# Kirkice/3DGaussian

Measured on AMD Instinct MI355X. Metric: Mpixels/sec fwd+bwd @1M Gaussians 800×800; PSNR vs torch ref, higher is better.
Workload: dtype f32 (splat contractions on v_mfma_f32_32x32x16_f16 with f32 accumulation; every operand in two round-to-nearest f16 pieces, pre-scaled into f16's normal range, three piece products: <= 3*2^-22 per product, forward and backward; no-depth-gradient mode); 1 GPU; C4: 1000000 Gaussians, 50 orbit views 800x800, fwd+bwd+grad all-reduce+Adam per step; gaussians=1000000, views=50, width=800, height=800, tile=32, seed=0, parallelism=view-sharded dp1, gaussian_order=morton (trainer layout, re-established every 16 steps)

## Files before the change

### 3dgaussian_amd/csrc/gr_hip.hip

```cpp

#include <hip/hip_runtime.h>
#include <hipcub/hipcub.hpp>
#include <rocprim/rocprim.hpp>

#include <cmath>
#include <cstdint>
#include <cstdio>
#include <cstdlib>
#include <cstring>
#include <atomic>
#include <mutex>
#include <string>
#include <vector>

#include "../../include/gr_hip.h"

#ifndef GR_TAIL2
#define GR_TAIL2 1
#endif
#ifndef GR_DEBUG_PREP_REPS
#define GR_DEBUG_PREP_REPS 1
#endif
#ifndef GR_DEBUG_BIN_REPS
#define GR_DEBUG_BIN_REPS 1
// ... 165 lines not shown
#pragma unroll
      for (int i = 4; i < 16; ++i)
#pragma unroll
        for (int k = 0; k < 3; ++k) out[k] += col[3 * i + k] * Y[i];
    }
  }
}

__device__ __forceinline__ float clamp01(float x) { return x < 0.0f ? 0.0f : (x > 1.0f ? 1.0f : x); }

__device__ __forceinline__ int tile_rect(const ViewK& v, const Proj& p, float op, int4& r) {
  r = make_int4(0, 0, -1, -1);
  if (!p.valid || !(op >= 0.0f)) return 0;
  const float R = v.cutoff;
  const float rx = R * p.sx, ry = R * p.sy;
  const float lox = p.px - rx, hix = p.px + rx, loy = p.py - ry, hiy = p.py + ry;
  const float wm1 = (float)(v.W - 1), hm1 = (float)(v.H - 1);
  if (!(hix >= 0.0f) || !(lox <= wm1) || !(hiy >= 0.0f) || !(loy <= hm1)) return 0;
  const int x0 = (lox <= 0.0f) ? 0 : (int)floorf(lox);
  const int x1 = (hix >= wm1) ? (v.W - 1) : (int)ceilf(hix);
  const int y0 = (loy <= 0.0f) ? 0 : (int)floorf(loy);
  const int y1 = (hiy >= hm1) ? (v.H - 1) : (int)ceilf(hiy);
  r = make_int4(x0 >> v.ts, y0 >> v.ts, x1 >> v.ts, y1 >> v.ts);
  r.y = max(r.y, v.ty0);
  r.w = min(r.w, v.ty1 - 1);
  if (r.y > r.w) {
    r = make_int4(0, 0, -1, -1);
    return 0;
  }
  return (r.z - r.x + 1) * (r.w - r.y + 1);
}

__device__ __forceinline__ float tile_emax(const ViewK& v, float px, float py, float qx, float qy, int tx, int ty) {
  const int xe = min(tx * v.T + v.T - 1, v.W - 1), ye = min(ty * v.T + v.T - 1, v.H - 1);
  const float lox = (float)(tx * v.T) + 0.5f, hix = (float)xe + 0.5f;
  const float loy = (float)(ty * v.T) + 0.5f, hiy = (float)ye + 0.5f;
  const float cx = px < lox ? lox : (px > hix ? hix : px);
  const float cy = py < loy ? loy : (py > hiy ? hiy : py);
  const float dx = cx - px, dy = cy - py;
  return (dx * dx) * qx + (dy * dy) * qy;
}

__device__ __forceinline__ float radius_thr(float R) { return (-0.5f * LOG2E) * (R * R); }

__device__ __forceinline__ float tile_ex(const ViewK& v, float px, float qx, int tx) {
  const int xe = min(tx * v.T + v.T - 1, v.W - 1);
  const float lox = (float)(tx * v.T) + 0.5f, hix = (float)xe + 0.5f;
  const float cx = px < lox ? lox : (px > hix ? hix : px);
  const float dx = cx - px;
  return (dx * dx) * qx;
}
__device__ __forceinline__ float tile_ey(const ViewK& v, float py, float qy, int ty) {
  const int ye = min(ty * v.T + v.T - 1, v.H - 1);
  const float loy = (float)(ty * v.T) + 0.5f, hiy = (float)ye + 0.5f;
  const float cy = py < loy ? loy : (py > hiy ? hiy : py);
  const float dy = cy - py;
  return (dy * dy) * qy;
}
__device__ __forceinline__ int tile_class_e(float e, float thr_cut, float thr_core) {
  return !(e >= thr_cut) ? 0 : (e >= thr_core ? 2 : 1);
}

__device__ __forceinline__ bool tile_pass(const ViewK& v, float px, float py, float qx, float qy, int tx, int ty) {
  return tile_emax(v, px, py, qx, qy, tx, ty) >= radius_thr(v.cutoff);
}

__device__ __forceinline__ int tile_class(const ViewK& v, float px, float py, float qx, float qy, int tx, int ty) {
  const float e = tile_emax(v, px, py, qx, qy, tx, ty);
  if (!(e >= radius_thr(v.cutoff))) return 0;
  return e >= radius_thr(v.core) ? 2 : 1;
}

__device__ __forceinline__ float qcoef(float s) { return (-0.5f * LOG2E) / (s * s); }


constexpr int REC4 = 2;

struct Cnt2 {
  unsigned long long v;
  __host__ __device__ unsigned c() const { return (unsigned)(v & 0xffffffffull); }
  __host__ __device__ unsigned t() const { return (unsigned)(v >> 32); }
};

struct Geom {
  float4* rec;
  float* zr;
  int4* rect;
  unsigned long long* counts;
  unsigned long long* offsets;
  gr_plan* plan;
  unsigned long long* total;
  float* omax;
  int* f16_sa;
  void* scan_tmp;
  size_t scan_tmp_bytes;
};

size_t geom_fixed(int n, size_t off[GR_GEOM_PARTS]) {
  size_t o = 0;
  const size_t nn = (size_t)(n > 0 ? n : 1);
  off[0] = o; o = align_up(o + (nn + 1) * (REC4 * sizeof(float4) + sizeof(float)));
  off[1] = o; o = align_up(o + nn * sizeof(int4));
  off[2] = o; o = align_up(o + (nn + 1) * sizeof(unsigned long long));
  off[3] = o; o = align_up(o + (nn + 1) * sizeof(unsigned long long));
  off[4] = o; o = align_up(o + sizeof(gr_plan) + (nn / 256 + 2) * (sizeof(unsigned long long) + sizeof(float)) + 16);
  off[5] = o;
  return o;
}

template <typename CountT>
size_t scan_tmp_bytes_t(int n) {
  size_t tmp = 0;
  (void)hipcub::DeviceScan::ExclusiveSum(nullptr, tmp, (CountT*)nullptr, (CountT*)nullptr, n + 1, (hipStream_t)0);
  return tmp;
}
size_t scan_tmp_bytes(int n) { return scan_tmp_bytes_t<unsigned long long>(n); }

Geom geom_view(void* base, int n) {
  size_t off[GR_GEOM_PARTS];
  const size_t fixed = geom_fixed(n, off);
  char* b = (char*)base;
  Geom g;
  g.plan = (gr_plan*)(b + off[4]);
  g.rec = (float4*)(b + off[0]);
  g.zr = (float*)(g.rec + (size_t)REC4 * ((size_t)n + 1));
  g.rect = (int4*)(b + off[1]);
  g.counts = (unsigned long long*)(b + off[2]);
  g.offsets = (unsigned long long*)(b + off[3]);
  g.total = (unsigned long long*)(b + off[4] + sizeof(gr_plan));
  g.omax = (float*)(g.total + (size_t)n / 256 + 2);
  g.f16_sa = (int*)(g.omax + (size_t)n / 256 + 2);
  g.scan_tmp = b + fixed;
  g.scan_tmp_bytes = 0;
  return g;
}

#ifndef GR_CH
#define GR_CH 2048
#endif
constexpr int CH = GR_CH;
#ifndef GR_CH32
#define GR_CH32 2048
#endif
constexpr int CH32 = GR_CH32;
constexpr int NPART = 9;

constexpr int TSORT_MAX_TILES = 16384;

inline bool short_keys(int tiles) { return tiles <= TSORT_MAX_TILES; }

struct Bins {
  uint32_t* keys;
  int* pairs;
  int2* ranges;
  int4* items;
  int* num_items;
  int* tile_item0;
  int* pos_of;
  int* ticket;
};

struct Scratch {
  uint32_t* keys_in;
  int* ids_in;
  float* fwd_part;
  int2* pairs_in;
  int2* pairs_sorted;
  void* sort_tmp;
};

inline int64_t item_cap(int tiles, int64_t K, int ch = CH) { return (K + ch - 1) / ch + tiles; }
constexpr int UF32_FRAGS = 2 * 4 * 2 * 2 * 64;
constexpr int UF32_STRIDE = UF32_FRAGS + 64;
struct TileCfg {
  int T, ch;
  size_t part_floats, uf_frags;
};
constexpr int UF_FRAGS16 = 2 * 3 * 3 * 64;
static int64_t tune_env(const char* name);
inline int chunk_of(const gr_view* v, int base, int64_t K) {
  static const int64_t force = tune_env("GR_TUNE_CHUNK");
  int64_t c = base;
  if (v->chunk > 0) {
    c = v->chunk;
  } else if (force > 0) {
    c = force;
  } else if (K >= 0) {
    c = 512;
    while (c < base && 2 * c * 1024 <= K) c *= 2;
  }
  return (int)std::min<int64_t>(8192, std::max<int64_t>(64, (c + 63) / 64 * 64));
}
inline TileCfg tile_cfg(const gr_view* v, int64_t K = -1) {
  return tile_of(v) == T32 ? TileCfg{T32, chunk_of(v, CH32, K), (size_t)4 * TP32, (size_t)UF32_STRIDE}
                           : TileCfg{T, chunk_of(v, CH, K), (size_t)5 * TP, (size_t)UF_FRAGS16};
}

constexpr int FAN_STRIDE = 32;
__host__ __device__ inline size_t fan_offset(int tiles) { return ((size_t)tiles + 1 + FAN_STRIDE - 1) / FAN_STRIDE * FAN_STRIDE; }

size_t bins_fixed(int vtiles, int64_t K, size_t off[8], int ch = CH) {
  const int tiles = vtiles;
  const size_t kk = (size_t)(K > 0 ? K : 1);
  const size_t cap = (size_t)item_cap(tiles, K, ch);
  size_t o = 0;
  off[0] = o; o = align_up(o + (short_keys(tiles) ? 1 : kk) * sizeof(uint32_t));
  off[1] = o; o = align_up(o + kk * sizeof(int));
  off[2] = o; o = align_up(o + (size_t)tiles * sizeof(int2));
  off[3] = o; o = align_up(o + cap * sizeof(int4));
  off[4] = o; o = align_up(o + 2 * sizeof(int));
  off[5] = o; o = align_up(o + (size_t)tiles * sizeof(int));
// ... 92 lines not shown
  r.keys_in = (uint32_t*)(b + off[0]);
  r.ids_in = (int*)(b + off[1]);
  r.fwd_part = (float*)(b + off[2]);
  r.pairs_in = (int2*)(b + off[3]);
  r.pairs_sorted = (int2*)(b + off[4]);
  r.sort_tmp = b + fixed;
  return r;
}

template <int NW>
__device__ __forceinline__ unsigned long long block_exclusive_scan(unsigned long long x, unsigned long long* sh,
                                                                   unsigned long long& total) {
  const int lane = (int)threadIdx.x & 63, w = (int)threadIdx.x >> 6;
  unsigned long long inc = x;
#pragma unroll
  for (int o = 1; o < 64; o <<= 1) {
    const unsigned long long y = __shfl_up(inc, o);
    if (lane >= o) inc += y;
  }
  __syncthreads();
  if (lane == 63) sh[w] = inc;
  __syncthreads();
  unsigned long long base = 0, all = 0;
#pragma unroll
  for (int u = 0; u < NW; ++u) {
    base += u < w ? sh[u] : 0ull;
    all += sh[u];
  }
  total = all;
  return base + inc - x;
}

template <int CD>
__device__ __forceinline__ unsigned long long preprocess_one(const ViewK& v, int i, const float* __restrict__ means,
                                                             const float* __restrict__ scales,
                                                             const float* __restrict__ colors,
                                                             const float* __restrict__ opac, Geom& g);

template <int CD>
__global__ __launch_bounds__(256) void k_preprocess(ViewK v, int n, const float* __restrict__ means,
                                                    const float* __restrict__ scales, const float* __restrict__ colors,
                                                    const float* __restrict__ opac, Geom g) {
  const int i = blockIdx.x * blockDim.x + threadIdx.x;
  if (i == n) {
    g.counts[n] = 0ull;
    float4* pad = g.rec + (size_t)REC4 * n;
    pad[0] = make_float4(1e30f, 1e30f, -1.0f, -1.0f);
    pad[1] = make_float4(0.f, 0.f, 0.f, 0.f);
    g.zr[n] = 0.0f;
  }
  unsigned long long kept = 0;
  if (i < n) kept = preprocess_one<CD>(v, i, means, scales, colors, opac, g);
  float om = kept != 0 ? g.rec[(size_t)REC4 * i + 1].x * fmaxf(1.0f, g.zr[i]) : 0.0f;
  __shared__ unsigned long long wsum[4];
  __shared__ float wmax[4];
#pragma unroll
  for (int m = 1; m < 64; m <<= 1) {
    kept += __shfl_xor(kept, m);
    om = fmaxf(om, __shfl_xor(om, m));
  }
  if ((threadIdx.x & 63) == 0) {
    wsum[threadIdx.x >> 6] = kept;
    wmax[threadIdx.x >> 6] = om;
  }
  __syncthreads();
  if (threadIdx.x == 0) {
    g.total[blockIdx.x] = (wsum[0] + wsum[1]) + (wsum[2] + wsum[3]);
    g.omax[blockIdx.x] = fmaxf(fmaxf(wmax[0], wmax[1]), fmaxf(wmax[2], wmax[3]));
  }
}

template <int CD>
__device__ __forceinline__ unsigned long long preprocess_vals(const ViewK& v, int i, float mx, float my, float mz, float s0,
                                                              float s1, const float* __restrict__ col, float op,
                                                              const Geom& g) {
  Proj p;
  project(v, mx, my, mz, s0, s1, p);
  float c[3];
  eval_color<CD>(v, mx, my, mz, col, c);
  int4 r;
  const float qx = qcoef(p.sx);
  const float qy = qcoef(p.sy);
  int core = 0, tail = 0;
  const int area = tile_rect(v, p, op, r);
  if (area > 0) {
    const float thr_cut = radius_thr(v.cutoff), thr_core = radius_thr(v.core);
    for (int ty = r.y; ty <= r.w; ++ty) {
      const float ey = tile_ey(v, p.py, qy, ty);
      for (int tx = r.x; tx <= r.z; ++tx) {
        const int cls = tile_class_e(tile_ex(v, p.px, qx, tx) + ey, thr_cut, thr_core);
        core += cls == 2;
        tail += cls == 1;
      }
    }
  }
  float4* rec = g.rec + (size_t)REC4 * i;
  rec[0] = make_float4(p.px, p.py, qx, qy);
  rec[1] = make_float4(op < 0.0f ? 0.0f : op, clamp01(c[0]), clamp01(c[1]), clamp01(c[2]));
  g.zr[i] = p.za;
  g.rect[i] = r;
  g.counts[i] = (unsigned long long)core | ((unsigned long long)tail << 32);
  return (unsigned long long)core | ((unsigned long long)tail << 32);
}

template <int CD>
__device__ __forceinline__ unsigned long long preprocess_one(const ViewK& v, int i, const float* __restrict__ means,
                                                             const float* __restrict__ scales,
                                                             const float* __restrict__ colors,
                                                             const float* __restrict__ opac, Geom& g) {
  return preprocess_vals<CD>(v, i, means[3 * i], means[3 * i + 1], means[3 * i + 2], scales[3 * i], scales[3 * i + 1],
                             colors + (size_t)CD * i, opac[i], g);
}

constexpr int PREP_MAX_VIEWS = GR_PREPARE_MAX_VIEWS;
struct PrepBatch {
  int nv;
  ViewK v[PREP_MAX_VIEWS];
  Geom g[PREP_MAX_VIEWS];
};

template <int CD>
__global__ __launch_bounds__(256) void k_preprocess_views(PrepBatch B, int n, const float* __restrict__ means,
                                                          const float* __restrict__ scales,
                                                          const float* __restrict__ colors,
                                                          const float* __restrict__ opac) {
  const int i = blockIdx.x * blockDim.x + threadIdx.x;
  float mx = 0.f, my = 0.f, mz = 0.f, s0 = 0.f, s1 = 0.f, op = 0.f;
  if (i < n) {
    mx = means[3 * i];
    my = means[3 * i + 1];
    mz = means[3 * i + 2];
    s0 = scales[3 * i];
    s1 = scales[3 * i + 1];
    op = opac[i];
  }
  __shared__ unsigned long long wsum[PREP_MAX_VIEWS][4];
  __shared__ float wmax[PREP_MAX_VIEWS][4];
  for (int k = blockIdx.y; k < B.nv; k += gridDim.y) {
    const Geom& g = B.g[k];
    if (i == n) {
      g.counts[n] = 0ull;
      float4* pad = g.rec + (size_t)REC4 * n;
      pad[0] = make_float4(1e30f, 1e30f, -1.0f, -1.0f);
      pad[1] = make_float4(0.f, 0.f, 0.f, 0.f);
      g.zr[n] = 0.0f;
    }
    unsigned long long kept = 0;
    if (i < n) kept = preprocess_vals<CD>(B.v[k], i, mx, my, mz, s0, s1, colors + (size_t)CD * i, op, g);
    float om = kept != 0 ? fmaxf(op, 0.0f) * fmaxf(1.0f, g.zr[i]) : 0.0f;
#pragma unroll
    for (int m = 1; m < 64; m <<= 1) {
      kept += __shfl_xor(kept, m);
      om = fmaxf(om, __shfl_xor(om, m));
    }
    if ((threadIdx.x & 63) == 0) {
      wsum[k][threadIdx.x >> 6] = kept;
      wmax[k][threadIdx.x >> 6] = om;
    }
  }
  __syncthreads();
  if ((int)threadIdx.x < B.nv && (int)threadIdx.x % (int)gridDim.y == (int)blockIdx.y) {
    const int k = threadIdx.x;
    B.g[k].total[blockIdx.x] = (wsum[k][0] + wsum[k][1]) + (wsum[k][2] + wsum[k][3]);
    B.g[k].omax[blockIdx.x] = fmaxf(fmaxf(wmax[k][0], wmax[k][1]), fmaxf(wmax[k][2], wmax[k][3]));
  }
}

constexpr int EWIN = 4096;

template <typename KeyT, typename OffT>
__global__ __launch_bounds__(256) void k_emit(ViewK v, int n, const int4* __restrict__ rect,
                                              const OffT* __restrict__ counts, const OffT* __restrict__ offsets,
                                              const KeyT* __restrict__ low_keys, KeyT* keys, int* ids) {
  __shared__ KeyT sK[EWIN];
  __shared__ int sI[EWIN];
  const int g0 = blockIdx.x * 256;
  const int i = g0 + (int)threadIdx.x;
  const int gend = min(n, g0 + 256);
  const int k0 = (int)(offsets[g0] & 0xffffffffu), k1 = (int)(offsets[gend] & 0xffffffffu);
  const bool staged = (k1 - k0) <= EWIN;
  if (i < n && counts[i] != 0) {
    const int4 r = rect[i];
    int k = (int)(offsets[i] & 0xffffffffu);
    const KeyT low = low_keys ? low_keys[i] : (KeyT)0;
// ... 7 lines not shown
          key = t;
        if (staged) {
          sK[k - k0] = key;
          sI[k - k0] = i;
        } else {
          keys[k] = key;
          ids[k] = i;
        }
        ++k;
      }
  }
  if (!staged) return;
  __syncthreads();
  for (int e = (int)threadIdx.x; e < k1 - k0; e += 256) {
    keys[k0 + e] = sK[e];
    ids[k0 + e] = sI[e];
  }
}

template <typename KeyT, bool VKEY>
__global__ __launch_bounds__(256) void k_emit_zones(ViewK v, int n, const int4* __restrict__ rect,
                                                    const Cnt2* __restrict__ counts, const Cnt2* __restrict__ offsets,
                                                    const float4* __restrict__ rec, KeyT* keys, int* ids) {
  __shared__ KeyT sK[EWIN];
  __shared__ int sI[EWIN];
  const int g0 = blockIdx.x * 256;
  const int i = g0 + (int)threadIdx.x;
  const int gend = min(n, g0 + 256);
  const int Kc = (int)offsets[n].c();
  const int c0 = (int)offsets[g0].c(), c1 = (int)offsets[gend].c();
  const int t0 = (int)offsets[g0].t(), t1 = (int)offsets[gend].t();
  const int nc = c1 - c0;
  const bool staged = nc + (t1 - t0) <= EWIN;
  if (i < n && counts[i].v != 0) {
    const int4 r = rect[i];
    const float4 a = rec[(size_t)REC4 * i];
    int kc = (int)offsets[i].c(), kt = (int)offsets[i].t();
    for (int ty = r.y; ty <= r.w; ++ty)
      for (int tx = r.x; tx <= r.z; ++tx) {
        const int cls = tile_class(v, a.x, a.y, a.z, a.w, tx, ty);
        if (cls == 0) continue;
        const int t = ty * v.tiles_x + tx;
        const KeyT key = (KeyT)(VKEY ? 2 * t + (cls == 1) : t);
        const int e = cls == 2 ? kc++ - c0 : nc + (kt++ - t0);
        if (staged) {
          sK[e] = key;
          sI[e] = i;
        } else {
          const int k = e < nc ? c0 + e : Kc + t0 + (e - nc);
          keys[k] = key;
          ids[k] = i;
        }
      }
  }
  if (!staged) return;
  __syncthreads();
  const int ne = nc + (t1 - t0);
  for (int e = (int)threadIdx.x; e < ne; e += 256) {
    const int k = e < nc ? c0 + e : Kc + t0 + (e - nc);
    keys[k] = sK[e];
    ids[k] = sI[e];
  }
}

constexpr int GR_BATCH_MAX = 8;
struct BI {
  int x, y;
};
template <class A>
struct VBatch {
  int nv;
  int first[GR_BATCH_MAX + 1];
  int gx[GR_BATCH_MAX];
  A a[GR_BATCH_MAX];
};
template <class A>
__device__ __forceinline__ int vbatch_view(const VBatch<A>& B, int b) {
  int v = 0;
  while (v + 1 < B.nv && b >= B.first[v + 1]) ++v;
  return v;
}

constexpr int EWIN_BLK = 4096;
__device__ __forceinline__ void k_emit_offsets_body(ViewK v, int n, const int4* __restrict__ rect, const Cnt2* __restrict__ counts,
                                                      const unsigned long long* __restrict__ bsum, Cnt2* __restrict__ offsets,
                                                      const float4* __restrict__ rec, uint16_t* __restrict__ keys,
                                                      int* __restrict__ ids, int* __restrict__ fan, const BI blockIdx, const BI gridDim) {
  __shared__ int sI[EWIN_BLK];
  __shared__ uint16_t sK[EWIN_BLK];
  __shared__ unsigned long long wsum[4];
  const int tid = threadIdx.x, b = blockIdx.x, i = b * 256 + tid;
  if (b == 0 && tid < 9) fan[FAN_STRIDE * tid] = 0;
  if (offsets[n].v == 0ull) {
    if (i < n) offsets[i].v = 0ull;
    return;
  }
  const Cnt2 cn{i < n ? counts[i].v : 0ull};
  const Cnt2 cb{bsum[b]};
  const int Kc = (int)offsets[n].c();
  const int4 rc = i < n ? rect[i] : make_int4(0, 0, -1, -1);
  const float4 a = i < n ? rec[(size_t)REC4 * i] : make_float4(0.f, 0.f, 0.f, 0.f);
  unsigned long long tot;
  const unsigned long long ex = block_exclusive_scan<4>(cn.v, wsum, tot);
  const int c0 = (int)cb.c(), t0 = (int)cb.t();
  const int nc = (int)(tot & 0xffffffffull), nt = (int)(tot >> 32);
  const bool staged = nc + nt <= EWIN_BLK;
  const unsigned long long run = cb.v + ex;
  if (i < n) offsets[i].v = run;
  if (cn.v != 0) {
    int kc = (int)(run & 0xffffffffull), kt = (int)(run >> 32);
    const float thr_cut = radius_thr(v.cutoff), thr_core = radius_thr(v.core);
    for (int ty = rc.y; ty <= rc.w; ++ty) {
      const float ey = tile_ey(v, a.y, a.w, ty);
      for (int tx = rc.x; tx <= rc.z; ++tx) {
        const int cls = tile_class_e(tile_ex(v, a.x, a.z, tx) + ey, thr_cut, thr_core);
        if (cls == 0) continue;
        const int t = ty * v.tiles_x + tx;
        const int e = cls == 2 ? kc++ - c0 : nc + (kt++ - t0);
        if (staged) {
          sK[e] = (uint16_t)t;
          sI[e] = i;
        } else {
          const int k = e < nc ? c0 + e : Kc + t0 + (e - nc);
          keys[k] = (uint16_t)t;
          ids[k] = i;
        }
      }
    }
  }
  if (!staged) return;
  __syncthreads();
  for (int e = tid; e < nc + nt; e += 256) {
    const int k = e < nc ? c0 + e : Kc + t0 + (e - nc);
    keys[k] = sK[e];
    ids[k] = sI[e];
  }
}
__global__ __launch_bounds__(256) void k_emit_offsets(ViewK v, int n, const int4* __restrict__ rect, const Cnt2* __restrict__ counts,
                                                      const unsigned long long* __restrict__ bsum, Cnt2* __restrict__ offsets,
                                                      const float4* __restrict__ rec, uint16_t* __restrict__ keys,
                                                      int* __restrict__ ids, int* __restrict__ fan) {
  k_emit_offsets_body(v, n, rect, counts, bsum, offsets, rec, keys, ids, fan, BI{(int)blockIdx.x, (int)blockIdx.y}, BI{(int)gridDim.x, (int)gridDim.y});
}
struct k_emit_offsets_args {
  ViewK v;
  int n;
  const int4* rect;
  const Cnt2* counts;
  const unsigned long long* bsum;
  Cnt2* offsets;
  const float4* rec;
  uint16_t* keys;
  int* ids;
  int* fan;
};
__global__ __launch_bounds__(256) void k_emit_offsets_views(VBatch<k_emit_offsets_args> B) {
  const int vb = vbatch_view(B, (int)blockIdx.x);
  const k_emit_offsets_args& a = B.a[vb];
  const int lb = (int)blockIdx.x - B.first[vb], gx = B.gx[vb];
  k_emit_offsets_body(a.v, a.n, a.rect, a.counts, a.bsum, a.offsets, a.rec, a.keys, a.ids, a.fan, BI{lb % gx, lb / gx}, BI{gx, (B.first[vb + 1] - B.first[vb]) / gx});
}


__global__ __launch_bounds__(256) void k_pos_of(int64_t K, const int2* __restrict__ sorted, int* __restrict__ ids,
                                                int* __restrict__ pos_of) {
  const int64_t k = (int64_t)blockIdx.x * blockDim.x + threadIdx.x;
  if (k >= K) return;
  const int2 p = sorted[k];
  ids[k] = p.x;
  pos_of[p.y] = (int)k;
}

__global__ __launch_bounds__(256) void k_pair_values(int64_t K, const int* __restrict__ ids, int2* __restrict__ pairs) {
  const int64_t k = (int64_t)blockIdx.x * blockDim.x + threadIdx.x;
  if (k < K) pairs[k] = make_int2(ids[k], (int)k);
}

template <typename KeyT>
__global__ __launch_bounds__(256) void k_ranges(int64_t K, const KeyT* __restrict__ keys, int2* ranges) {
  const int64_t k = (int64_t)blockIdx.x * blockDim.x + threadIdx.x;
  if (k >= K) return;
  const int shift = sizeof(KeyT) == 8 ? 32 : 0;
  const int t = (int)(keys[k] >> shift);
  if (k == 0 || (int)(keys[k - 1] >> shift) != t) ranges[t].x = (int)k;
  if (k == K - 1 || (int)(keys[k + 1] >> shift) != t) ranges[t].y = (int)(k + 1);
}

typedef float f32x4 __attribute__((ext_vector_type(4)));

#ifndef GR_WI_THREADS
#define GR_WI_THREADS 256
#endif
constexpr int WI_THREADS = GR_WI_THREADS;
__device__ __forceinline__ int chunks_of(int len, int ch) { return (len + ch - 1) / ch; }
__global__ __launch_bounds__(WI_THREADS) void k_work_items(int vtiles, const int2* __restrict__ ranges, int4* __restrict__ items,
                                                     int* __restrict__ num_items, int* __restrict__ tile_item0,
                                                     int* __restrict__ ticket, int ch) {
  typedef hipcub::BlockScan<int, WI_THREADS> Scan;
  __shared__ typename Scan::TempStorage tmp;
  __shared__ int carry;
  const int tiles = vtiles / 2;
  for (int pass = 0; pass < 2; ++pass) {
    if (threadIdx.x == 0 && pass == 0) carry = 0;
    __syncthreads();
    for (int base = 0; base < tiles; base += WI_THREADS) {
      const int t = base + (int)threadIdx.x;
      const int2 rc = t < tiles ? ranges[2 * t] : make_int2(0, 0), rt = t < tiles ? ranges[2 * t + 1] : make_int2(0, 0);
      const int chc = chunks_of(rc.y - rc.x, ch), cht = chunks_of(rt.y - rt.x, ch);
      const int nch = t >= tiles ? 0 : pass == 0 ? chc + cht : (chc + cht == 0 ? 1 : 0);
      int excl, total;
      Scan(tmp).ExclusiveSum(nch, excl, total);
      const int first = carry + excl;
      if (t < tiles && pass == 0) {
        ticket[t] = 0;
        tile_item0[2 * t] = first;
        tile_item0[2 * t + 1] = first + chc;
        for (int c = 0; c < chc; ++c) items[first + c] = make_int4(2 * t, rc.x + c * ch, min(rc.y, rc.x + (c + 1) * ch), c);
        for (int c = 0; c < cht; ++c)
          items[first + chc + c] = make_int4(2 * t + 1, rt.x + c * ch, min(rt.y, rt.x + (c + 1) * ch), c);
      } else if (nch) {
        tile_item0[2 * t] = tile_item0[2 * t + 1] = first;
        items[first] = make_int4(2 * t, 0, 0, 0);
      }
      __syncthreads();
      if (threadIdx.x == 0) carry += total;
      __syncthreads();
    }
    if (threadIdx.x == 0) num_items[1 - pass] = carry;
  }
  if (threadIdx.x < 9) ticket[fan_offset(tiles) + FAN_STRIDE * threadIdx.x] = 0;
}

__device__ __forceinline__ int stage_id(int k, int k1, const int* __restrict__ pairs) { return pairs[min(k, k1 - 1)]; }
__device__ __forceinline__ int stage_pair(int raw, int k, int k1) { return k < k1 ? raw : -1; }

typedef __attribute__((address_space(3))) void* lds_ptr_t;

__device__ __forceinline__ uint32_t lds_addr(void* p) {
  return __builtin_amdgcn_readfirstlane((uint32_t)(uintptr_t)(lds_ptr_t)p);
}
__device__ __forceinline__ void glds16(const void* gsrc, void* wave_base) {
  unsigned keep;
  asm volatile("s_mov_b32 %0, m0\n\ts_mov_b32 m0, %2\n\ts_nop 0\n\tglobal_load_lds_dwordx4 %1, off\n\ts_mov_b32 m0, %0"
// ... 4021 lines not shown
                                     const float* scales, const float* colors, int color_dim, const float* opacities,
                                     void* const* geoms, size_t geom_bytes, const gr_plan* caps, gr_plan* const* observed,
                                     int* overflow, void* stream) {
  if (!caps) return set_error(GR_ERR_INVALID_ARGUMENT, "gr_fwd_prepare_views_sized: caps is null");
  return prepare_views_impl(num_views, views, n, means, scales, colors, color_dim, opacities, geoms, geom_bytes, observed,
                            caps, overflow, stream);
}

gr_status gr_fwd_prepare(const gr_view* v, int n, const float* means, const float* scales, const float* colors,
                         int color_dim, const float* opacities, void* geom, size_t geom_bytes, gr_plan* plan,
                         void* stream) {
  if (plan) {
    plan->num_pairs = 0;
    plan->num_slots = 0;
    plan->num_core_pairs = 0;
  }
  gr_status st = gr_fwd_prepare_async(v, n, means, scales, colors, color_dim, opacities, geom, geom_bytes, plan, stream);
  if (st != GR_OK || n == 0) return st;
  GR_HIP_TRY(hipStreamSynchronize((hipStream_t)stream));
  if (plan->num_pairs < 0) return set_error(GR_ERR_OVERFLOW, "pair count overflows int32");
  return GR_OK;
}

}

struct BwdWs {
  float* partials;
  uint4* UF;
  float* tile_loss;
  float* tile_aux;
  float* dscal;
  float* sums;
  float* sums3;
  double* cam_part;
};
static BwdWs bwd_ws(const gr_view* v, int n, const gr_plan* plan, void* ws) {
  const size_t tiles = (size_t)tiles_of(v);
  BwdWs w;
  w.partials = (float*)ws;
  w.UF = (uint4*)((char*)ws + align_up((size_t)(plan->num_slots > 0 ? plan->num_slots : 1) * NPART * sizeof(float)));
  w.tile_loss = (float*)((char*)w.UF + align_up(tiles * tile_cfg(v).uf_frags * sizeof(uint4)));
  w.tile_aux = (float*)((char*)w.tile_loss + align_up(tiles * 4 * sizeof(float)));
  w.dscal = (float*)((char*)w.tile_aux + align_up(tiles * 2 * sizeof(float)));
  w.sums = (float*)((char*)w.dscal + align_up(4 * sizeof(float)));
  w.sums3 = (float*)((char*)w.sums + align_up((size_t)8 * (n > 0 ? n : 1) * sizeof(float)));
  w.cam_part = (double*)((char*)w.sums3 + align_up((size_t)(n > 0 ? n : 1) * sizeof(float)));
  return w;
}

static gr_status bin_impl(const gr_view* v, int n, const gr_plan* plan, const void* geom, const Bins& b,
                          const Scratch& sc, const ViewK& vk, hipStream_t s) {
  const int64_t num_pairs = plan->num_pairs;
  const int tiles = vk.tiles_x * vk.tiles_y, vtiles = 2 * tiles;
  prof_mark(PROF_BINNING, s);
  if (n > 0 && num_pairs > 0) {
    Geom g = geom_view((void*)geom, n);
    const Cnt2* cnt = (const Cnt2*)g.counts;
    const Cnt2* offs = (const Cnt2*)g.offsets;
    if (short_keys(vtiles)) {
      const int64_t Kc = plan->num_core_pairs, Kr[2] = {Kc, num_pairs - Kc};
      const int cw = col_width(num_pairs, tiles);
      const size_t cells = (size_t)tiles * cols_of(num_pairs, cw);
      const int waves = tsort_waves(tiles);
      TZones Z;
      Z.cw = cw;
      Z.ch = tile_cfg(v, num_pairs).ch;
      Z.kdev = v->device_counts ? (const unsigned long long*)(g.offsets + n) : nullptr;
      char* q = (char*)sc.sort_tmp;
      for (int z = 0; z < 2; ++z) {
        TZone& zz = Z.z[z];
        zz.K = Kr[z];
        zz.cols = cols_of(Kr[z], cw);
        zz.zbase = z == 0 ? 0 : (int)Kc;
        zz.keys = (const uint16_t*)sc.keys_in + (z == 0 ? 0 : Kc);
        zz.ids = sc.ids_in + (z == 0 ? 0 : Kc);
        zz.M = (int*)q;
        q += align_up(cells * sizeof(int));
        zz.S = (int*)q;
        q += align_up(cells * sizeof(int));
        zz.T = (int*)q;
        q += align_up((size_t)tiles * sizeof(int));
      }
      int* fan = b.ticket + fan_offset(tiles);
      hipLaunchKernelGGL(k_emit_offsets, dim3(blocks_for(n)), dim3(256), 0, s, vk, n, (const int4*)g.rect, cnt,
                         (const unsigned long long*)g.total, (Cnt2*)g.offsets, (const float4*)g.rec,
                         (uint16_t*)sc.keys_in, sc.ids_in, fan);
      GR_HIP_TRY(hipGetLastError());
      const int blocks = Z.z[0].cols + Z.z[1].cols;
      hipLaunchKernelGGL(k_tile_count, dim3(blocks), dim3(256), (size_t)tiles * sizeof(int), s, Z, tiles);
      GR_HIP_TRY(hipGetLastError());
      hipLaunchKernelGGL(k_tile_colscan, dim3((tiles + CS_T - 1) / CS_T, 2), dim3(CS_T * CS_G), 0, s, Z, tiles, b.ranges,
                         b.items, b.num_items, b.tile_item0, b.ticket);
      GR_HIP_TRY(hipGetLastError());
      const size_t lds = (size_t)tiles * sizeof(int) * waves;
      const int bits = bits_for((uint32_t)tiles);
      if (waves == 8)
        hipLaunchKernelGGL(k_tile_place<8>, dim3(blocks), dim3(512), lds, s, Z, tiles, bits, (const int2*)b.ranges, b.pairs,
                           b.pos_of);
      else if (waves == 4)
        hipLaunchKernelGGL(k_tile_place<4>, dim3(blocks), dim3(256), lds, s, Z, tiles, bits, (const int2*)b.ranges, b.pairs,
                           b.pos_of);
      else if (waves == 2)
        hipLaunchKernelGGL(k_tile_place<2>, dim3(blocks), dim3(128), lds, s, Z, tiles, bits, (const int2*)b.ranges, b.pairs,
                           b.pos_of);
      else
        hipLaunchKernelGGL(k_tile_place<1>, dim3(blocks), dim3(64), lds, s, Z, tiles, bits, (const int2*)b.ranges, b.pairs,
                           b.pos_of);
      GR_HIP_TRY(hipGetLastError());
    } else {
      if (v->device_counts)
        return set_error(GR_ERR_INVALID_ARGUMENT, "device_counts views need the counting-sort binning (<= 8,192 tiles)");
      hipLaunchKernelGGL(k_offsets, dim3(blocks_for(n)), dim3(256), 0, s, n, (const unsigned long long*)g.counts,
                         (const unsigned long long*)g.total, g.offsets);
      GR_HIP_TRY(hipGetLastError());
      hipLaunchKernelGGL((k_emit_zones<uint32_t, true>), dim3(blocks_for(n)), dim3(256), 0, s, vk, n,
                         (const int4*)g.rect, cnt, offs, (const float4*)g.rec, sc.keys_in, sc.ids_in);
      GR_HIP_TRY(hipGetLastError());
      hipLaunchKernelGGL(k_pair_values, dim3(blocks_for(num_pairs)), dim3(256), 0, s, num_pairs, (const int*)sc.ids_in,
                         sc.pairs_in);
      GR_HIP_TRY(hipGetLastError());
      GR_HIP_TRY(hipMemsetAsync(b.ranges, 0, sizeof(int2) * vtiles, s));
      const int bits = bits_for((uint32_t)vtiles);
      size_t tmp = tile_sort_tmp_bytes(n, num_pairs, vtiles);
      GR_HIP_TRY(hipcub::DeviceRadixSort::SortPairs(sc.sort_tmp, tmp, sc.keys_in, b.keys, sc.pairs_in, sc.pairs_sorted,
                                                    (int)num_pairs, 0, bits, s));
      hipLaunchKernelGGL(k_ranges<uint32_t>, dim3(blocks_for(num_pairs)), dim3(256), 0, s, num_pairs, b.keys, b.ranges);
      GR_HIP_TRY(hipGetLastError());
      hipLaunchKernelGGL(k_pos_of, dim3(blocks_for(num_pairs)), dim3(256), 0, s, num_pairs, (const int2*)sc.pairs_sorted,
                         b.pairs, b.pos_of);
      GR_HIP_TRY(hipGetLastError());
      hipLaunchKernelGGL(k_work_items, dim3(1), dim3(WI_THREADS), 0, s, vtiles, (const int2*)b.ranges, b.items, b.num_items,
                         b.tile_item0, b.ticket, tile_cfg(v, num_pairs).ch);
    }
  } else {
    if (n > 0) GR_HIP_TRY(hipMemsetAsync(geom_view((void*)geom, n).offsets, 0, (size_t)n * sizeof(unsigned long long), s));
    GR_HIP_TRY(hipMemsetAsync(b.ranges, 0, sizeof(int2) * vtiles, s));
    hipLaunchKernelGGL(k_work_items, dim3(1), dim3(WI_THREADS), 0, s, vtiles, (const int2*)b.ranges, b.items, b.num_items,
                       b.tile_item0, b.ticket, tile_cfg(v, num_pairs).ch);
  }
  GR_HIP_TRY(hipGetLastError());
  prof_mark(PROF_BINNING, s);
  return GR_OK;
}

static gr_status fwd_impl(const gr_view* v, int n, const gr_plan* plan, const void* geom, void* bins, size_t bins_bytes,
                          void* scratch, size_t scratch_bytes, float* out_rgb, float* out_alpha, float* out_depth,
                          float* saved, void* stream, const L1Args* l1, float* l1_loss_out, void* ws, size_t ws_bytes,
                          bool depth_sums = false) {
  gr_status st = check_view(v);
  if (st != GR_OK) return st;
  if (!plan) return set_error(GR_ERR_INVALID_ARGUMENT, "plan is null");
  if (plan->num_pairs < 0 || plan->num_slots < 0) return set_error(GR_ERR_OVERFLOW, "pair count overflows int32");
  if (!l1 && !saved) return set_error(GR_ERR_INVALID_ARGUMENT, "saved is required");
  if (l1 && (!ws || ws_bytes < gr_bwd_bytes(v, n, plan) || !l1_loss_out))
    return set_error(GR_ERR_WORKSPACE, "gr_fwd_render_l1: backward workspace too small (or null loss)");
  if (n > 0 && (!geom || !bins)) return set_error(GR_ERR_INVALID_ARGUMENT, "null workspace");
  const int64_t num_pairs = plan->num_pairs;
  if (bins_bytes < gr_bins_bytes(v, n, plan)) return set_error(GR_ERR_WORKSPACE, "bins workspace too small");
  if (scratch_bytes < gr_fwd_scratch_bytes(v, n, plan) || !scratch)
    return set_error(GR_ERR_WORKSPACE, "forward scratch workspace too small");
  hipStream_t s = (hipStream_t)stream;
  const ViewK vk = make_viewk(v);
  const int tiles = vk.tiles_x * vk.tiles_y, vtiles = 2 * tiles;
  const TileCfg tc = tile_cfg(v, num_pairs);
  if (v->rows > 0 && !l1)
    return set_error(GR_ERR_INVALID_ARGUMENT, "a band of tile rows (gr_view.rows): gr_fwd_render_l1 only (the fit loss)");
  if (tc.T == T32 && (!l1 || v->no_depth_grad != 1))
    return set_error(GR_ERR_INVALID_ARGUMENT, "32-pixel tiles (gr_view.tile = 32): gr_fwd_render_l1 with no_depth_grad = 1 only");
  if (tc.T == T32 && vk.core != vk.cutoff)
// ... 353 lines not shown
  B.first[0] = 0;
  return B;
}
#define GR_VB_LAUNCH(kern, B, threads, lds, s)                                                   \
  do {                                                                                           \
    if ((B).first[(B).nv] > 0) {                                                                 \
      hipLaunchKernelGGL(kern, dim3((unsigned)(B).first[(B).nv]), dim3(threads), lds, s, (B));   \
      GR_HIP_TRY(hipGetLastError());                                                             \
    }                                                                                            \
  } while (0)

extern "C" {

gr_status gr_fit_views_batched(int num_views, const gr_batch_view* bv, int n, float w_sil, float w_depth,
                                          float g_scale, void* stream) {
  if (num_views < 1 || num_views > GR_BATCH_MAX_VIEWS || !bv)
    return set_error(GR_ERR_INVALID_ARGUMENT, "gr_fit_views_batched: num_views must be in [1, GR_BATCH_MAX_VIEWS]");
  if (n <= 0) return set_error(GR_ERR_INVALID_ARGUMENT, "gr_fit_views_batched: n must be > 0");
  static_assert(GR_BATCH_MAX_VIEWS == GR_BATCH_MAX, "gr_hip.h GR_BATCH_MAX_VIEWS");
  const gr_view& v0 = bv[0].view;
  const bool depth = bv[0].target_depth != nullptr;
  for (int j = 0; j < num_views; ++j) {
    const gr_batch_view& b = bv[j];
    gr_status st = check_view(&b.view);
    if (st != GR_OK) return st;
    if (b.view.width != v0.width || b.view.height != v0.height || tile_of(&b.view) != tile_of(&v0) ||
        b.view.no_depth_grad != v0.no_depth_grad || b.view.cutoff != v0.cutoff || b.view.core_cutoff != v0.core_cutoff ||
        b.view.device_counts != v0.device_counts || (b.target_depth != nullptr) != depth)
      return set_error(GR_ERR_INVALID_ARGUMENT, "gr_fit_views_batched: the views differ in size, tile, footprint or mode");
    if (b.plan.num_pairs <= 0 || b.plan.num_slots < b.plan.num_pairs)
      return set_error(GR_ERR_INVALID_ARGUMENT, "gr_fit_views_batched: every view needs pairs (or capacities)");
    if (!b.geom || !b.bins || !b.scratch || !b.ws || !b.target_rgb || !b.sums || !b.loss || (depth && (!b.saved || !b.sums3)))
      return set_error(GR_ERR_INVALID_ARGUMENT, "gr_fit_views_batched: null pointer");
    if (b.bins_bytes < gr_bins_bytes(&b.view, n, &b.plan) || b.scratch_bytes < gr_fwd_scratch_bytes(&b.view, n, &b.plan) ||
        b.ws_bytes < gr_bwd_bytes(&b.view, n, &b.plan))
      return set_error(GR_ERR_WORKSPACE, "gr_fit_views_batched: a workspace is too small");
  }
  if (!short_keys(vtiles_of(&v0)))
    return set_error(GR_ERR_INVALID_ARGUMENT, "gr_fit_views_batched: more than 8,192 screen tiles");
  if (depth ? v0.no_depth_grad != 0 : v0.no_depth_grad != 1)
    return set_error(GR_ERR_INVALID_ARGUMENT, "gr_fit_views_batched: depth loss needs no_depth_grad = 0, the L1 path 1");
  if (depth && tile_of(&v0) != T)
    return set_error(GR_ERR_INVALID_ARGUMENT, "gr_fit_views_batched: the depth-loss path runs at 16-pixel tiles");
  for (int j = 0; j < num_views && depth; ++j)
    if (bv[j].view.rows > 0)
      return set_error(GR_ERR_INVALID_ARGUMENT, "gr_fit_views_batched: a band of tile rows needs the L1 path (no depth loss)");
  hipStream_t s = (hipStream_t)stream;
  const int tiles = vtiles_of(&v0) / 2;
  const size_t HW = (size_t)v0.width * v0.height;
  const int waves = tsort_waves(tiles), bits = bits_for((uint32_t)tiles);
  auto Be = vb_new<k_emit_offsets_args>();
  auto Bc = vb_new<k_tile_count_args>();
  auto Bs = vb_new<k_tile_colscan_args>();
  auto Bp = vb_new<k_tile_place_args>();
  for (int j = 0; j < num_views; ++j) {
    const gr_batch_view& b = bv[j];
    const ViewK vk = make_viewk(&b.view);
    const TileCfg tc = tile_cfg(&b.view, b.plan.num_pairs);
    const Bins bn = bins_view(b.bins, 2 * tiles, b.plan.num_pairs, tc.ch);
    const Scratch sc = scratch_view(b.scratch, 2 * tiles, b.plan.num_pairs, tc.ch, tc.part_floats);
    Geom g = geom_view((void*)b.geom, n);
    const int64_t K = b.plan.num_pairs, Kc = b.plan.num_core_pairs, Kr[2] = {Kc, K - Kc};
    TZones Z;
    Z.cw = col_width(K, tiles);
    Z.ch = tc.ch;
    Z.kdev = b.view.device_counts ? (const unsigned long long*)(g.offsets + n) : nullptr;
    const size_t cells = (size_t)tiles * cols_of(K, Z.cw);
    char* q = (char*)sc.sort_tmp;
    for (int z = 0; z < 2; ++z) {
      TZone& zz = Z.z[z];
      zz.K = Kr[z];
      zz.cols = cols_of(Kr[z], Z.cw);
      zz.zbase = z == 0 ? 0 : (int)Kc;
      zz.keys = (const uint16_t*)sc.keys_in + (z == 0 ? 0 : Kc);
      zz.ids = sc.ids_in + (z == 0 ? 0 : Kc);
      zz.M = (int*)q;
      q += align_up(cells * sizeof(int));
      zz.S = (int*)q;
      q += align_up(cells * sizeof(int));
      zz.T = (int*)q;
      q += align_up((size_t)tiles * sizeof(int));
    }
    const int cols = Z.z[0].cols + Z.z[1].cols;
    vb_add(Be, k_emit_offsets_args{vk, n, (const int4*)g.rect, (const Cnt2*)g.counts, (const unsigned long long*)g.total,
                                   (Cnt2*)g.offsets, (const float4*)g.rec, (uint16_t*)sc.keys_in, sc.ids_in,
                                   bn.ticket + fan_offset(tiles)},
           blocks_for(n));
    vb_add(Bc, k_tile_count_args{Z, tiles}, cols);
    const int gxs = (tiles + CS_T - 1) / CS_T;
    vb_add(Bs, k_tile_colscan_args{Z, tiles, bn.ranges, bn.items, bn.num_items, bn.tile_item0, bn.ticket}, 2 * gxs, gxs);
    vb_add(Bp, k_tile_place_args{Z, tiles, bits, (const int2*)bn.ranges, bn.pairs, bn.pos_of}, cols);
  }
  GR_VB_LAUNCH(k_emit_offsets_views, Be, 256, 0, s);
  GR_VB_LAUNCH(k_tile_count_views, Bc, 256, (size_t)tiles * sizeof(int), s);
  GR_VB_LAUNCH(k_tile_colscan_views, Bs, CS_T * CS_G, 0, s);
  const size_t lds = (size_t)tiles * sizeof(int) * waves;
  if (waves == 8) GR_VB_LAUNCH(k_tile_place_views<8>, Bp, 512, lds, s);
  else if (waves == 4) GR_VB_LAUNCH(k_tile_place_views<4>, Bp, 256, lds, s);
  else if (waves == 2) GR_VB_LAUNCH(k_tile_place_views<2>, Bp, 128, lds, s);
  else GR_VB_LAUNCH(k_tile_place_views<1>, Bp, 64, lds, s);

  auto Bg = vb_new<k_gather_view_args>();
  if (!depth) {
    auto Bf = vb_new<k_fwd32_l1_args>();
    auto Bf16 = vb_new<k_raster_fwd_mfma_args>();
    auto Bb = vb_new<k_bwd32_args>();
    auto Bb16 = vb_new<k_raster_bwd_bf16_args>();
    for (int j = 0; j < num_views; ++j) {
      const gr_batch_view& b = bv[j];
      const ViewK vk = make_viewk(&b.view);
      const TileCfg tc = tile_cfg(&b.view, b.plan.num_pairs);
      const Bins bn = bins_view(b.bins, 2 * tiles, b.plan.num_pairs, tc.ch);
      const Scratch sc = scratch_view(b.scratch, 2 * tiles, b.plan.num_pairs, tc.ch, tc.part_floats);
      const Geom g = geom_view((void*)b.geom, n);
      const BwdWs w = bwd_ws(&b.view, n, &b.plan, b.ws);
      L1Args la{b.target_rgb, b.target_mask, w_sil, g_scale, w.tile_loss};
      la.pieces = 2;
      la.loss_out = b.loss;
      la.n1 = (int64_t)(3 * HW);
      la.n2 = (int64_t)(b.target_mask ? HW : 0);
      const int cap = (int)item_cap(2 * tiles, b.plan.num_pairs, tc.ch);
      if (tc.T == T32) {
        vb_add(Bf, k_fwd32_l1_args{vk, n, (const int4*)bn.items, (const int*)bn.num_items, (const int2*)bn.ranges,
                                   (const int*)bn.pairs, (const float4*)g.rec, sc.fwd_part, nullptr, nullptr, la, w.UF,
                                   (const int*)g.f16_sa, (const int*)bn.tile_item0, bn.ticket, tc.ch},
               cap);
        vb_add(Bb, k_bwd32_args{vk, n, (const int4*)bn.items, (const int*)bn.num_items, (const int*)bn.pairs,
                                (const float4*)g.rec, (const uint4*)w.UF, w.partials},
               cap);
      } else {
        vb_add(Bf16, k_raster_fwd_mfma_args{vk, n, (const int4*)bn.items, (const int*)bn.num_items, (const int2*)bn.ranges,
                                            (const int*)bn.pairs, (const float4*)g.rec, sc.fwd_part, nullptr, nullptr,
                                            nullptr, nullptr, nullptr, la, w.UF, (const int*)g.f16_sa,
                                            (const int*)bn.tile_item0, bn.ticket, tc.ch},
               cap);
        vb_add(Bb16, k_raster_bwd_bf16_args{vk, n, (const int4*)bn.items, (const int*)bn.num_items, (const int*)bn.pairs,
                                            (const float4*)g.rec, (const uint4*)w.UF, w.partials, nullptr},
               cap);
      }
      vb_add(Bg, k_gather_view_args{n, (const Cnt2*)g.offsets, (const int*)bn.pos_of, (const float4*)w.partials,
                                    (float2*)b.sums, nullptr, nullptr},
             (n + 63) / 64);
    }
    GR_VB_LAUNCH(k_fwd32_l1_views, Bf, 256, 0, s);
    GR_VB_LAUNCH(k_raster_fwd_mfma_views<4>, Bf16, 256, 0, s);
    GR_VB_LAUNCH(k_bwd32_views, Bb, 256, 0, s);
    GR_VB_LAUNCH((k_raster_bwd_bf16_views<false, 2>), Bb16, 256, 0, s);
    GR_VB_LAUNCH(k_gather_view_views<false>, Bg, 256, 0, s);
    return GR_OK;
  }
  auto Bf = vb_new<k_raster_fwd_mfma_args>();
  auto Bm = vb_new<k_depth_tile_max_args>();
  auto Bd = vb_new<k_depth_tile_sums_args>();
  auto Bu = vb_new<k_pixel_grads_args>();
  auto Bb = vb_new<k_raster_bwd_bf16_args>();
  for (int j = 0; j < num_views; ++j) {
    const gr_batch_view& b = bv[j];
    const ViewK vk = make_viewk(&b.view);
    const TileCfg tc = tile_cfg(&b.view, b.plan.num_pairs);
    const Bins bn = bins_view(b.bins, 2 * tiles, b.plan.num_pairs, tc.ch);
    const Scratch sc = scratch_view(b.scratch, 2 * tiles, b.plan.num_pairs, tc.ch, tc.part_floats);
    const Geom g = geom_view((void*)b.geom, n);
    const BwdWs w = bwd_ws(&b.view, n, &b.plan, b.ws);
    float4* s4 = (float4*)b.saved;
    float* sD = b.saved + 4 * HW;
    const int cap = (int)item_cap(2 * tiles, b.plan.num_pairs, tc.ch);
    L1Args none{nullptr, nullptr, 0.f, 0.f, nullptr};
// ... 710 lines not shown
```

Before: 1524 Mpixels/sec.

## Cache per-Gaussian tile classification bitmasks from preprocess for key emission

Preprocess now records, for Gaussians covering at most 32 tiles, two 32-bit bitplanes marking core and tail tiles. Larger footprints store a flagged count so emission falls back to recomputation. Emission derives counts by popcount and walks the set bits to write keys, instead of re-evaluating the Gaussian falloff per tile and reloading the record. This adds an extra 8-byte mask array per Gaussian per view, an extra store in preprocess, and a slight geometry-buffer size increase.

```diff
diff --git a/3dgaussian_amd/csrc/gr_hip.hip b/3dgaussian_amd/csrc/gr_hip.hip
--- a/3dgaussian_amd/csrc/gr_hip.hip
+++ b/3dgaussian_amd/csrc/gr_hip.hip
@@ -271,12 +271,29 @@
   __host__ __device__ unsigned t() const { return (unsigned)(v >> 32); }
 };
 
+struct TileMask {
+  static constexpr int TILES = 32;
+  static constexpr unsigned long long MARK = 0x100000001ull;
+  __host__ __device__ static unsigned long long planes(unsigned core, unsigned tail) {
+    return (unsigned long long)core | ((unsigned long long)tail << 32);
+  }
+  __host__ __device__ static unsigned long long recompute(int core, int tail) {
+    return MARK | planes((unsigned)core << 1, (unsigned)tail << 1);
+  }
+  __host__ __device__ static bool is_recompute(unsigned long long m) { return (m & MARK) == MARK; }
+  __device__ static unsigned long long counts(unsigned long long m) {
+    const unsigned lo = (unsigned)m, hi = (unsigned)(m >> 32);
+    return is_recompute(m) ? planes(lo >> 1, hi >> 1) : planes((unsigned)__popc(lo), (unsigned)__popc(hi));
+  }
+};
+
 struct Geom {
   float4* rec;
   float* zr;
   int4* rect;
   unsigned long long* counts;
   unsigned long long* offsets;
+  unsigned long long* mask;
   gr_plan* plan;
   unsigned long long* total;
   float* omax;
@@ -292,6 +309,7 @@
   off[1] = o; o = align_up(o + nn * sizeof(int4));
   off[2] = o; o = align_up(o + (nn + 1) * sizeof(unsigned long long));
   off[3] = o; o = align_up(o + (nn + 1) * sizeof(unsigned long long));
+  o = align_up(o + nn * sizeof(unsigned long long));
   off[4] = o; o = align_up(o + sizeof(gr_plan) + (nn / 256 + 2) * (sizeof(unsigned long long) + sizeof(float)) + 16);
   off[5] = o;
   return o;
@@ -316,6 +334,7 @@
   g.rect = (int4*)(b + off[1]);
   g.counts = (unsigned long long*)(b + off[2]);
   g.offsets = (unsigned long long*)(b + off[3]);
+  g.mask = (unsigned long long*)(b + off[3] + align_up(((size_t)(n > 0 ? n : 1) + 1) * sizeof(unsigned long long)));
   g.total = (unsigned long long*)(b + off[4] + sizeof(gr_plan));
   g.omax = (float*)(g.total + (size_t)n / 256 + 2);
   g.f16_sa = (int*)(g.omax + (size_t)n / 256 + 2);
@@ -574,9 +593,10 @@
   const float qx = qcoef(p.sx);
   const float qy = qcoef(p.sy);
   int core = 0, tail = 0;
+  unsigned long long mask = 0ull;
   const int area = tile_rect(v, p, op, r);
-  if (area > 0) {
-    const float thr_cut = radius_thr(v.cutoff), thr_core = radius_thr(v.core);
+  const float thr_cut = radius_thr(v.cutoff), thr_core = radius_thr(v.core);
+  if (area > TileMask::TILES) {
     for (int ty = r.y; ty <= r.w; ++ty) {
       const float ey = tile_ey(v, p.py, qy, ty);
       for (int tx = r.x; tx <= r.z; ++tx) {
@@ -585,6 +605,22 @@
         tail += cls == 1;
       }
     }
+    mask = TileMask::recompute(core, tail);
+  } else if (area > 0) {
+    unsigned cut = 0u, cor = 0u, bit = 1u;
+    for (int ty = r.y; ty <= r.w; ++ty) {
+      const float ey = tile_ey(v, p.py, qy, ty);
+      for (int tx = r.x; tx <= r.z; ++tx) {
+        const float e = tile_ex(v, p.px, qx, tx) + ey;
+        cut |= e >= thr_cut ? bit : 0u;
+        cor |= e >= thr_core ? bit : 0u;
+        bit <<= 1;
+      }
+    }
+    const unsigned cp = cut & cor, tp = cut & ~cor;
+    core = __popc(cp);
+    tail = __popc(tp);
+    mask = TileMask::planes(cp, tp);
   }
   float4* rec = g.rec + (size_t)REC4 * i;
   rec[0] = make_float4(p.px, p.py, qx, qy);
@@ -592,6 +628,7 @@
   g.zr[i] = p.za;
   g.rect[i] = r;
   g.counts[i] = (unsigned long long)core | ((unsigned long long)tail << 32);
+  g.mask[i] = mask;
   return (unsigned long long)core | ((unsigned long long)tail << 32);
 }
 
@@ -765,7 +802,7 @@
 }
 
 constexpr int EWIN_BLK = 4096;
-__device__ __forceinline__ void k_emit_offsets_body(ViewK v, int n, const int4* __restrict__ rect, const Cnt2* __restrict__ counts,
+__device__ __forceinline__ void k_emit_offsets_body(ViewK v, int n, const int4* __restrict__ rect, const unsigned long long* __restrict__ mask,
                                                       const unsigned long long* __restrict__ bsum, Cnt2* __restrict__ offsets,
                                                       const float4* __restrict__ rec, uint16_t* __restrict__ keys,
                                                       int* __restrict__ ids, int* __restrict__ fan, const BI blockIdx, const BI gridDim) {
@@ -778,11 +815,11 @@
     if (i < n) offsets[i].v = 0ull;
     return;
   }
-  const Cnt2 cn{i < n ? counts[i].v : 0ull};
+  const unsigned long long m = i < n ? mask[i] : 0ull;
   const Cnt2 cb{bsum[b]};
   const int Kc = (int)offsets[n].c();
   const int4 rc = i < n ? rect[i] : make_int4(0, 0, -1, -1);
-  const float4 a = i < n ? rec[(size_t)REC4 * i] : make_float4(0.f, 0.f, 0.f, 0.f);
+  const Cnt2 cn{TileMask::counts(m)};
   unsigned long long tot;
   const unsigned long long ex = block_exclusive_scan<4>(cn.v, wsum, tot);
   const int c0 = (int)cb.c(), t0 = (int)cb.t();
@@ -790,25 +827,44 @@
   const bool staged = nc + nt <= EWIN_BLK;
   const unsigned long long run = cb.v + ex;
   if (i < n) offsets[i].v = run;
-  if (cn.v != 0) {
-    int kc = (int)(run & 0xffffffffull), kt = (int)(run >> 32);
-    const float thr_cut = radius_thr(v.cutoff), thr_core = radius_thr(v.core);
-    for (int ty = rc.y; ty <= rc.w; ++ty) {
-      const float ey = tile_ey(v, a.y, a.w, ty);
-      for (int tx = rc.x; tx <= rc.z; ++tx) {
-        const int cls = tile_class_e(tile_ex(v, a.x, a.z, tx) + ey, thr_cut, thr_core);
-        if (cls == 0) continue;
-        const int t = ty * v.tiles_x + tx;
-        const int e = cls == 2 ? kc++ - c0 : nc + (kt++ - t0);
-        if (staged) {
-          sK[e] = (uint16_t)t;
-          sI[e] = i;
-        } else {
-          const int k = e < nc ? c0 + e : Kc + t0 + (e - nc);
-          keys[k] = (uint16_t)t;
-          ids[k] = i;
+  int kc = (int)(run & 0xffffffffull), kt = (int)(run >> 32);
+  auto put = [&](int cls, int t) {
+    const int e = cls == 2 ? kc++ - c0 : nc + (kt++ - t0);
+    if (staged) {
+      sK[e] = (uint16_t)t;
+      sI[e] = i;
+    } else {
+      const int k = e < nc ? c0 + e : Kc + t0 + (e - nc);
+      keys[k] = (uint16_t)t;
+      ids[k] = i;
+    }
+  };
+  if (TileMask::is_recompute(m)) {
+    if (cn.v != 0) {
+      const float4 a = rec[(size_t)REC4 * i];
+      const float thr_cut = radius_thr(v.cutoff), thr_core = radius_thr(v.core);
+      for (int ty = rc.y; ty <= rc.w; ++ty) {
+        const float ey = tile_ey(v, a.y, a.w, ty);
+        for (int tx = rc.x; tx <= rc.z; ++tx) {
+          const int cls = tile_class_e(tile_ex(v, a.x, a.z, tx) + ey, thr_cut, thr_core);
+          if (cls != 0) put(cls, ty * v.tiles_x + tx);
         }
       }
+    }
+  } else {
+    const int w = rc.z - rc.x + 1, skip = v.tiles_x - w;
+    int t0r = rc.y * v.tiles_x + rc.x, rowend = w;
+    const unsigned cp = (unsigned)m;
+    unsigned both = cp | (unsigned)(m >> 32);
+    while (both != 0u) {
+      const int j = __builtin_ctz(both);
+      const int cls = (cp >> j) & 1u ? 2 : 1;
+      both &= both - 1u;
+      while (j >= rowend) {
+        rowend += w;
+        t0r += skip;
+      }
+      put(cls, t0r + j);
     }
   }
   if (!staged) return;
@@ -819,17 +875,17 @@
     ids[k] = sI[e];
   }
 }
-__global__ __launch_bounds__(256) void k_emit_offsets(ViewK v, int n, const int4* __restrict__ rect, const Cnt2* __restrict__ counts,
+__global__ __launch_bounds__(256) void k_emit_offsets(ViewK v, int n, const int4* __restrict__ rect, const unsigned long long* __restrict__ mask,
                                                       const unsigned long long* __restrict__ bsum, Cnt2* __restrict__ offsets,
                                                       const float4* __restrict__ rec, uint16_t* __restrict__ keys,
                                                       int* __restrict__ ids, int* __restrict__ fan) {
-  k_emit_offsets_body(v, n, rect, counts, bsum, offsets, rec, keys, ids, fan, BI{(int)blockIdx.x, (int)blockIdx.y}, BI{(int)gridDim.x, (int)gridDim.y});
+  k_emit_offsets_body(v, n, rect, mask, bsum, offsets, rec, keys, ids, fan, BI{(int)blockIdx.x, (int)blockIdx.y}, BI{(int)gridDim.x, (int)gridDim.y});
 }
 struct k_emit_offsets_args {
   ViewK v;
   int n;
   const int4* rect;
-  const Cnt2* counts;
+  const unsigned long long* mask;
   const unsigned long long* bsum;
   Cnt2* offsets;
   const float4* rec;
@@ -841,7 +897,7 @@
   const int vb = vbatch_view(B, (int)blockIdx.x);
   const k_emit_offsets_args& a = B.a[vb];
   const int lb = (int)blockIdx.x - B.first[vb], gx = B.gx[vb];
-  k_emit_offsets_body(a.v, a.n, a.rect, a.counts, a.bsum, a.offsets, a.rec, a.keys, a.ids, a.fan, BI{lb % gx, lb / gx}, BI{gx, (B.first[vb + 1] - B.first[vb]) / gx});
+  k_emit_offsets_body(a.v, a.n, a.rect, a.mask, a.bsum, a.offsets, a.rec, a.keys, a.ids, a.fan, BI{lb % gx, lb / gx}, BI{gx, (B.first[vb + 1] - B.first[vb]) / gx});
 }
 
 
@@ -5029,9 +5085,9 @@
         q += align_up((size_t)tiles * sizeof(int));
       }
       int* fan = b.ticket + fan_offset(tiles);
-      hipLaunchKernelGGL(k_emit_offsets, dim3(blocks_for(n)), dim3(256), 0, s, vk, n, (const int4*)g.rect, cnt,
-                         (const unsigned long long*)g.total, (Cnt2*)g.offsets, (const float4*)g.rec,
-                         (uint16_t*)sc.keys_in, sc.ids_in, fan);
+      hipLaunchKernelGGL(k_emit_offsets, dim3(blocks_for(n)), dim3(256), 0, s, vk, n, (const int4*)g.rect,
+                         (const unsigned long long*)g.mask, (const unsigned long long*)g.total, (Cnt2*)g.offsets,
+                         (const float4*)g.rec, (uint16_t*)sc.keys_in, sc.ids_in, fan);
       GR_HIP_TRY(hipGetLastError());
       const int blocks = Z.z[0].cols + Z.z[1].cols;
       hipLaunchKernelGGL(k_tile_count, dim3(blocks), dim3(256), (size_t)tiles * sizeof(int), s, Z, tiles);
@@ -5551,7 +5607,7 @@
       q += align_up((size_t)tiles * sizeof(int));
     }
     const int cols = Z.z[0].cols + Z.z[1].cols;
-    vb_add(Be, k_emit_offsets_args{vk, n, (const int4*)g.rect, (const Cnt2*)g.counts, (const unsigned long long*)g.total,
+    vb_add(Be, k_emit_offsets_args{vk, n, (const int4*)g.rect, (const unsigned long long*)g.mask, (const unsigned long long*)g.total,
                                    (Cnt2*)g.offsets, (const float4*)g.rec, (uint16_t*)sc.keys_in, sc.ids_in,
                                    bn.ticket + fan_offset(tiles)},
            blocks_for(n));
```

After: 1532 Mpixels/sec, median of 6. No clear change (+0.5%).
